# jinhojsk515/spmm

Hardware: AMD Instinct MI355X
Metric: pretrain molecules/sec (higher is better)
Workload: dtype bf16; 1 GPU; SPMM pretrain step, text 12 layers (fusion at 6) + PV 6 layers, H=768, 12 heads, queue 36864, train mode (dropout 0.1), fwd+bwd+clip+AdamW+EMA; global_batch=128, seq_len=128, parallelism=dp1, schedule=eager launches on three HIP streams, packed text rows

## Files before the change

spmm_amd/csrc/gemm.hip:

```cpp
#include "common.h"
#include "../../include/spmm_hip.h"

namespace {

constexpr int BM = 128, BN = 128, BK = 64;
constexpr int TILE_BYTES = BM * BK * 2;
constexpr int STAGE_BYTES = 2 * TILE_BYTES;

enum Epi { EPI_BF16 = 0, EPI_GELU = 1, EPI_F32 = 2, EPI_F32_ATOMIC = 3, EPI_GELU_GRAD = 4, EPI_F32_ACC = 5, EPI_GELU_DERIV = 6, EPI_MUL = 7 };
constexpr bool epi_is_bf16(int e) { return e == EPI_BF16 || e == EPI_GELU || e == EPI_GELU_GRAD || e == EPI_GELU_DERIV || e == EPI_MUL; }

struct GemmP {
  const bf16* A; long lda;
  const bf16* W; long ldw;
  int M, N, K;
  int ksplit;
  const float* bias;
  const float* div_ptr;
  float alpha;
  const bf16* R; long ldr;
  const bf16* G; long ldg;
  void* C; long ldc;
  bf16* C2; long ldc2;
  float* colsum;
// ... 521 lines not shown
        if (p.R) {
          const bf16x4 r = *(const bf16x4*)(p.R + (long)m * p.ldr + n);
#pragma unroll
          for (int j = 0; j < 4; ++j) v[j] += (float)r[j];
        }
        if constexpr (EPI == EPI_BF16) {
          *(bf16x4*)((bf16*)p.C + (long)m * p.ldc + n) = to_bf16x4(v[0], v[1], v[2], v[3]);
        } else if constexpr (EPI == EPI_GELU) {
          *(bf16x4*)(p.C2 + (long)m * p.ldc2 + n) = to_bf16x4(v[0], v[1], v[2], v[3]);
          *(bf16x4*)((bf16*)p.C + (long)m * p.ldc + n) =
              to_bf16x4(gelu_erf(v[0]), gelu_erf(v[1]), gelu_erf(v[2]), gelu_erf(v[3]));
        } else if constexpr (EPI == EPI_GELU_GRAD) {
          const bf16x4 x = *(const bf16x4*)(p.G + (long)m * p.ldg + n);
          *(bf16x4*)((bf16*)p.C + (long)m * p.ldc + n) =
              to_bf16x4(v[0] * gelu_erf_grad((float)x[0]), v[1] * gelu_erf_grad((float)x[1]),
                        v[2] * gelu_erf_grad((float)x[2]), v[3] * gelu_erf_grad((float)x[3]));
        } else if constexpr (EPI == EPI_F32) {
          f32x4 o = {v[0], v[1], v[2], v[3]};
          *(f32x4*)((float*)p.C + (long)m * p.ldc + n) = o;
        } else {
          f32x4* dst = (f32x4*)((float*)p.C + (long)m * p.ldc + n);
          f32x4 o = *dst;
          o[0] += v[0]; o[1] += v[1]; o[2] += v[2]; o[3] += v[3];
          *dst = o;
        }
      }
    }
}

__device__ __forceinline__ void tile_of(int t, int ntm, int ntn, int order, int& tm, int& tn) {
  if (order == 1) { tn = t / ntm; tm = t - tn * ntm; return; }
  if (order == 2) {
    const int gn = (ntn % 4 == 0) ? 4 : (ntn % 3 == 0 ? 3 : (ntn % 2 == 0 ? 2 : 1));
    const int sr = t / (8 * ntn);
    const int rows = min(8, ntm - sr * 8);
    const int r = t - sr * 8 * ntn;
    const int nb = r / (rows * gn), rr = r - nb * rows * gn;
    tm = sr * 8 + rr % rows;
    tn = nb * gn + rr / rows;
    return;
  }
  if (order >= 3 && ntn >= 8) {
    const int ng = order == 3 ? 2 : 4, base = ntn / ng, rem = ntn - base * ng;
    int c0 = 0, u = t;
#pragma unroll
    for (int g = 0; g < 4; ++g) {
      if (g >= ng) break;
      const int cg = base + (g < rem ? 1 : 0), sz = ntm * cg;
      if (u < sz || g == ng - 1) { tm = u / cg; tn = c0 + (u - tm * cg); return; }
      u -= sz; c0 += cg;
    }
  }
  tm = t / ntn; tn = t - tm * ntn;
}

constexpr int BM3 = 256, BN3 = 256;
constexpr int T3_BYTES = 256 * BK * 2;
constexpr int STAGE3_BYTES = 2 * T3_BYTES;
constexpr int LDS3_BYTES = 2 * STAGE3_BYTES;

template <int EPI>
__global__ __launch_bounds__(512) void gemm_nt_v3_kernel(GemmP p) {
  extern __shared__ __attribute__((aligned(16))) char smem3[];
  const int tid = threadIdx.x, lane = tid & 63, wave = tid >> 6;
  const int wm = wave >> 2, wn = wave & 3;
  GEMM_DYN_M(p);
  const int ntm = (p.M + BM3 - 1) / BM3, ntn = (p.N + BN3 - 1) / BN3, nt = ntm * ntn;
  int t;
  {
    const int b = blockIdx.x, q = nt >> 3, r = nt & 7, xcd = b & 7, i = b >> 3;
    if (i >= (xcd < r ? q + 1 : q)) return;
    t = (xcd < r ? xcd * (q + 1) : r * (q + 1) + (xcd - r) * q) + i;
  }
  int tile_m, tile_n;
  tile_of(t, ntm, ntn, p.order, tile_m, tile_n);
  const int m0 = tile_m * BM3, n0 = tile_n * BN3;
  const int nk = p.K / BK;

  f32x16 acc[2][2][2];
#pragma unroll
  for (int h = 0; h < 2; ++h)
#pragma unroll
    for (int i = 0; i < 2; ++i)
#pragma unroll
      for (int j = 0; j < 2; ++j)
#pragma unroll
        for (int r = 0; r < 16; ++r) acc[h][i][j][r] = 0.f;

#define STAGE3(kt_)                                                                           \
  do {                                                                                        \
    char* b_ = smem3 + ((kt_) & 1) * STAGE3_BYTES;                                            \
    stage2_dma(p.A, p.lda, m0, p.M, (kt_) * BK, b_, tid, 4);                                  \
    stage2_dma(p.W, p.ldw, n0, p.N, (kt_) * BK, b_ + T3_BYTES, tid, 4);                       \
  } while (0)

  STAGE3(0);
  for (int kt = 0; kt < nk; ++kt) {
    __syncthreads();
    if (kt + 1 < nk) STAGE3(kt + 1);
    const char* As = smem3 + (kt & 1) * STAGE3_BYTES;
    const char* Ws = As + T3_BYTES;
#pragma unroll
    for (int kk = 0; kk < 4; ++kk) {
      const int s = kk * 2 + (lane >> 5);
      bf16x8 af[4], wf[2];
#pragma unroll
      for (int i = 0; i < 4; ++i) {
        const int ar = wm * 128 + i * 32 + (lane & 31);
        af[i] = *(const bf16x8*)(As + ar * 128 + ((s ^ ((ar >> 1) & 7)) << 4));
      }
#pragma unroll
      for (int i = 0; i < 2; ++i) {
        const int wr = wn * 64 + i * 32 + (lane & 31);
        wf[i] = *(const bf16x8*)(Ws + wr * 128 + ((s ^ ((wr >> 1) & 7)) << 4));
      }
#pragma unroll
      for (int h = 0; h < 2; ++h)
#pragma unroll
        for (int ni = 0; ni < 2; ++ni)
#pragma unroll
          for (int mi = 0; mi < 2; ++mi)
            acc[h][ni][mi] = __builtin_amdgcn_mfma_f32_32x32x16_bf16(wf[ni], af[h * 2 + mi], acc[h][ni][mi], 0, 0, 0);
    }
  }
#undef STAGE3
  __syncthreads();
  char* wt = smem3 + wave * 16384;
  float cs_carry[8] = {0.f, 0.f, 0.f, 0.f, 0.f, 0.f, 0.f, 0.f};
#pragma unroll
  for (int h = 0; h < 2; ++h)
    epilogue_bf16<EPI>(p, acc[h], wt, m0 + wm * 128 + h * 64, n0 + wn * 64, lane, cs_carry, h == 1);
}

constexpr int P8_HT = 128 * BK * 2;
constexpr int P8_BUF = 4 * P8_HT;
constexpr int P8_LDS = 2 * P8_BUF;
constexpr int P8_XLDS = 8 * 4096;

template <int OFF>
__device__ __forceinline__ void p8_dsr(bf16x8& d, uint32_t addr) {
  asm volatile("ds_read_b128 %0, %1 offset:%2" : "=v"(d) : "v"(addr), "n"(OFF) : "memory");
}

struct P8Out { uint32_t d[4]; };
__device__ __forceinline__ uint32_t p8_pack2(float a, float b) {
  typedef __bf16 bf16x2 __attribute__((ext_vector_type(2)));
  bf16x2 v; v[0] = (bf16)a; v[1] = (bf16)b;
  return __builtin_bit_cast(uint32_t, v);
}
__device__ __forceinline__ float p8_lo(uint32_t w) { return __builtin_bit_cast(float, w << 16); }
__device__ __forceinline__ float p8_hi(uint32_t w) { return __builtin_bit_cast(float, w & 0xffff0000u); }
typedef uint32_t u32x2 __attribute__((ext_vector_type(2)));
typedef uint32_t u32x4 __attribute__((ext_vector_type(4)));
template <int OFF>
__device__ __forceinline__ void p8_dsw64(uint32_t addr, uint32_t a, uint32_t b) {
  u32x2 v = {a, b};
  asm volatile("ds_write_b64 %0, %1 offset:%2" :: "v"(addr), "v"(v), "n"(OFF) : "memory");
}
template <int OFF>
__device__ __forceinline__ void p8_dsr128u(u32x4& d, uint32_t addr) {
  asm volatile("ds_read_b128 %0, %1 offset:%2" : "=v"(d) : "v"(addr), "n"(OFF) : "memory");
}

template <int EPI, bool INTERIOR, bool HAS_EX, typename Hook>
__device__ __forceinline__ void p8_epilogue_blocks(const GemmP& p, f32x4 (&acc)[2][4][4], uint32_t xb ,
                                                   int m_base, int n_base, int lane, Hook hook) {
  float scale = p.alpha;
  if (p.div_ptr) scale /= *p.div_ptr;
  const int m = lane & 15, g = lane >> 4, r8 = lane >> 3, c16 = lane & 7;
  f32x4 b[4];
#pragma unroll
  for (int ni = 0; ni < 4; ++ni) b[ni] = f32x4{0.f, 0.f, 0.f, 0.f};
  if (p.bias) {
#pragma unroll
    for (int ni = 0; ni < 4; ++ni)
      if (INTERIOR || n_base + ni * 16 + 4 * g < p.N) b[ni] = *(const f32x4*)(p.bias + n_base + ni * 16 + 4 * g);
  }
  uint32_t wad[4];
#pragma unroll
  for (int ni = 0; ni < 4; ++ni) wad[ni] = xb + (uint32_t)(m * 128 + ((((ni * 2 + (g >> 1)) ^ (m & 7)) << 4) | ((g & 1) << 3)));
  const uint32_t rad = xb + (uint32_t)(r8 * 128 + ((c16 ^ (r8 & 7)) << 4));
  const long n = n_base + c16 * 8;
  const bool n_ok = INTERIOR || n < p.N;
  const long row0 = m_base + r8;
  bf16* cp = (bf16*)p.C + row0 * p.ldc + n;
  constexpr bool GELU2 = EPI == EPI_GELU || EPI == EPI_GELU_DERIV;
  constexpr bool DERIV = EPI == EPI_GELU_DERIV;
  constexpr bool MULG = EPI == EPI_MUL;
  bf16* c2p = GELU2 && p.C2 ? p.C2 + row0 * p.ldc2 + n : nullptr;
  u32x4 ex[8];
  const bf16* esrc = (EPI == EPI_GELU_GRAD || MULG) ? p.G : p.R;
  const long eld = (EPI == EPI_GELU_GRAD || MULG) ? p.ldg : p.ldr;
  const long nn = n_ok ? n : 0;
#define P8_EX_LOAD1(I_, R_)                                                                                            \
  do {                                                                                                                 \
    ex[I_] = *(const u32x4*)(esrc + (R_) * eld + nn);                                                                  \
  } while (0)
#define P8_LOAD_EX(H)                                                          \
  if constexpr (HAS_EX) {                                                      \
    _Pragma("unroll") for (int i_ = 0; i_ < 8; ++i_) {                         \
      long r_ = row0 + (H) * 64 + i_ * 8;                                      \
      if (!INTERIOR) r_ = r_ < p.M ? r_ : p.M - 1;                             \
      P8_EX_LOAD1(i_, r_);                                                     \
    }                                                                          \
  }
  P8_LOAD_EX(0);
  float cs[8] = {0.f, 0.f, 0.f, 0.f, 0.f, 0.f, 0.f, 0.f};
#pragma unroll
  for (int h = 0; h < 2; ++h)
#pragma unroll
    for (int mi = 0; mi < 4; ++mi) {
      const int blk = h * 4 + mi;
      const uint32_t bo = (blk & 1) * 2048;
      const bool ok1 = INTERIOR || (n_ok && row0 + blk * 16 < p.M), ok2 = INTERIOR || (n_ok && row0 + blk * 16 + 8 < p.M);
      float v[4][4];
#pragma unroll
      for (int ni = 0; ni < 4; ++ni)
#pragma unroll
        for (int j = 0; j < 4; ++j) v[ni][j] = acc[h][mi][ni][j] * scale + b[ni][j];
#pragma unroll
      for (int ni = 0; ni < 4; ++ni) acc[h][mi][ni] = f32x4{0.f, 0.f, 0.f, 0.f};
      u32x4 o1, o2;
      if constexpr (GELU2) {
        float w[4][4];
#pragma unroll
        for (int ni = 0; ni < 4; ++ni)
#pragma unroll
          for (int j = 0; j < 4; j += 2) {
            const f32x2 x = {v[ni][j], v[ni][j + 1]};
            f32x2 gg, dd = x;
            gelu_erf_pair<DERIV>(x, gg, dd);
            v[ni][j] = gg.x; v[ni][j + 1] = gg.y;
            w[ni][j] = dd.x; w[ni][j + 1] = dd.y;
          }
        if (c2p) {
          u32x4 q1, q2;
#pragma unroll
          for (int ni = 0; ni < 4; ++ni) p8_dsw64<0>(wad[ni] + bo, p8_pack2(w[ni][0], w[ni][1]), p8_pack2(w[ni][2], w[ni][3]));
#pragma unroll
          for (int ni = 0; ni < 4; ++ni) p8_dsw64<0>(wad[ni] + (bo ^ 2048u), p8_pack2(v[ni][0], v[ni][1]), p8_pack2(v[ni][2], v[ni][3]));
          p8_dsr128u<0>(q1, rad + bo);
          p8_dsr128u<1024>(q2, rad + bo);
          p8_dsr128u<0>(o1, rad + (bo ^ 2048u));
          p8_dsr128u<1024>(o2, rad + (bo ^ 2048u));
          asm volatile("s_waitcnt lgkmcnt(0)" ::: "memory");
          __builtin_amdgcn_sched_barrier(0);
          if (ok1) *(u32x4*)(c2p + (long)blk * 16 * p.ldc2) = q1;
          if (ok2) *(u32x4*)(c2p + (long)blk * 16 * p.ldc2 + 8 * p.ldc2) = q2;
        }
      }
      if (!(GELU2 && c2p)) {
#pragma unroll
        for (int ni = 0; ni < 4; ++ni) p8_dsw64<0>(wad[ni] + bo, p8_pack2(v[ni][0], v[ni][1]), p8_pack2(v[ni][2], v[ni][3]));
        p8_dsr128u<0>(o1, rad + bo);
        p8_dsr128u<1024>(o2, rad + bo);
        asm volatile("s_waitcnt lgkmcnt(0)" ::: "memory");
        __builtin_amdgcn_sched_barrier(0);
      }
      if constexpr (EPI == EPI_BF16 && HAS_EX) {
#pragma unroll
        for (int d = 0; d < 4; ++d) {
          o1[d] = p8_pack2(p8_lo(o1[d]) + p8_lo(ex[2 * mi][d]), p8_hi(o1[d]) + p8_hi(ex[2 * mi][d]));
          o2[d] = p8_pack2(p8_lo(o2[d]) + p8_lo(ex[2 * mi + 1][d]), p8_hi(o2[d]) + p8_hi(ex[2 * mi + 1][d]));
        }
      }
      if constexpr (EPI == EPI_GELU_GRAD) {
#pragma unroll
        for (int d = 0; d < 4; ++d) {
          o1[d] = p8_pack2(p8_lo(o1[d]) * gelu_erf_grad(p8_lo(ex[2 * mi][d])), p8_hi(o1[d]) * gelu_erf_grad(p8_hi(ex[2 * mi][d])));
          o2[d] = p8_pack2(p8_lo(o2[d]) * gelu_erf_grad(p8_lo(ex[2 * mi + 1][d])), p8_hi(o2[d]) * gelu_erf_grad(p8_hi(ex[2 * mi + 1][d])));
        }
      }
      if constexpr (EPI == EPI_MUL) {
#pragma unroll
        for (int d = 0; d < 4; ++d) {
          o1[d] = p8_pack2(p8_lo(o1[d]) * p8_lo(ex[2 * mi][d]), p8_hi(o1[d]) * p8_hi(ex[2 * mi][d]));
          o2[d] = p8_pack2(p8_lo(o2[d]) * p8_lo(ex[2 * mi + 1][d]), p8_hi(o2[d]) * p8_hi(ex[2 * mi + 1][d]));
        }
      }
      if constexpr (!GELU2) {
        if (p.colsum) {
#pragma unroll
          for (int d = 0; d < 4; ++d) {
            if (ok1) { cs[2 * d] += p8_lo(o1[d]); cs[2 * d + 1] += p8_hi(o1[d]); }
            if (ok2) { cs[2 * d] += p8_lo(o2[d]); cs[2 * d + 1] += p8_hi(o2[d]); }
          }
        }
      }
#ifdef P8_NOSTORE
      if (p.M < 0) {
#endif
#ifdef P8_STORE_POLICY
      if (ok1) asm volatile("global_store_dwordx4 %0, %1, off " P8_STORE_POLICY :: "v"(cp + (long)blk * 16 * p.ldc), "v"(o1) : "memory");
      if (ok2) asm volatile("global_store_dwordx4 %0, %1, off " P8_STORE_POLICY :: "v"(cp + (long)blk * 16 * p.ldc + 8 * p.ldc), "v"(o2) : "memory");
#else
      if (ok1) *(u32x4*)(cp + (long)blk * 16 * p.ldc) = o1;
      if (ok2) *(u32x4*)(cp + (long)blk * 16 * p.ldc + 8 * p.ldc) = o2;
#endif
#ifdef P8_NOSTORE
      }
#endif
      hook(blk);
      if constexpr (HAS_EX && EPI == EPI_GELU_GRAD) {
        if (blk == 3) { P8_LOAD_EX(1); }
      } else if constexpr (HAS_EX) {
        if (h == 0) {
#pragma unroll
          for (int i_ = 2 * mi; i_ < 2 * mi + 2; ++i_) {
            long r_ = row0 + 64 + i_ * 8;
            if (!INTERIOR) r_ = r_ < p.M ? r_ : p.M - 1;
            P8_EX_LOAD1(i_, r_);
          }
        }
      }
    }
#undef P8_LOAD_EX
#undef P8_EX_LOAD1
  if constexpr (!GELU2) {
    if (p.colsum) {
#pragma unroll
      for (int e = 0; e < 8; ++e) {
        float t = cs[e];
        t += __shfl_xor(t, 8, 64);
        t += __shfl_xor(t, 16, 64);
        t += __shfl_xor(t, 32, 64);
        cs[e] = t;
      }
      if (lane < 8 && n_ok) {
#pragma unroll
        for (int e = 0; e < 8; ++e) atomicAdd(p.colsum + n + e, cs[e]);
      }
    }
  }
}

template <int EPI>
__global__ __launch_bounds__(512) void gemm_nt_p8_kernel(GemmP p) {
  extern __shared__ __attribute__((aligned(16))) char smem8[];
  const int tid = threadIdx.x, lane = tid & 63;
  const int wave = __builtin_amdgcn_readfirstlane(tid >> 6);
  const int wr = wave >> 2, wc = wave & 3;
  GEMM_DYN_M(p);
  const int ntm = (p.M + BM3 - 1) / BM3, ntn = (p.N + BN3 - 1) / BN3, nt = ntm * ntn;
  if ((int)blockIdx.x >= nt) return;
  const int nk = p.K / BK;

  f32x4 acc[2][4][4];
#define P8_ZERO()                                                              \
  _Pragma("unroll") for (int h_ = 0; h_ < 2; ++h_)                             \
  _Pragma("unroll") for (int i_ = 0; i_ < 4; ++i_)                             \
  _Pragma("unroll") for (int j_ = 0; j_ < 4; ++j_) acc[h_][i_][j_] = f32x4{0.f, 0.f, 0.f, 0.f}
  P8_ZERO();

  uint32_t offA[2][2], offW[2][2];
  const uint32_t ls16 = (uint32_t)(((tid & 7) ^ ((tid >> 4) & 7)) * 16);
  int m0, n0;
#define P8_TILE(VB)                                                                                           \
  do {                                                                                                        \
    const int b_ = (VB), q_ = nt >> 3, r_ = nt & 7, xcd_ = b_ & 7, i_ = b_ >> 3;                              \
    const int t_ = (xcd_ < r_ ? xcd_ * (q_ + 1) : r_ * (q_ + 1) + (xcd_ - r_) * q_) + i_;                     \
    int tm_, tn_;                                                                                             \
    tile_of(t_, ntm, ntn, p.order, tm_, tn_);                                                                 \
    m0 = tm_ * BM3; n0 = tn_ * BN3;                                                                           \
    _Pragma("unroll") for (int h_ = 0; h_ < 2; ++h_)                                                          \
    _Pragma("unroll") for (int j_ = 0; j_ < 2; ++j_) {                                                        \
      int row_ = m0 + j_ * 128 + h_ * 64 + (tid >> 3);                                                        \
      row_ = row_ < p.M ? row_ : p.M - 1;                     \
      offA[h_][j_] = (uint32_t)row_ * (uint32_t)(p.lda * 2) + ls16;                                                      \
      int col_ = n0 + (j_ * 2 + (tid >> 8)) * 64 + h_ * 32 + ((tid >> 3) & 31);                               \
      col_ = col_ < p.N ? col_ : p.N - 1;                                                                     \
      offW[h_][j_] = (uint32_t)col_ * (uint32_t)(p.ldw * 2) + ls16;                                                      \
    }                                                                                                         \
  } while (0)
  const char* gA = (const char*)p.A;
  const char* gW = (const char*)p.W;
  const uint32_t lds0 = (uint32_t)(uintptr_t)(LDS_AS char*)smem8;
#define P8_STG(GB, O, SLOT)                                                                                               \
  do {                                                                                                                    \
    const uint32_t d_ = lds0 + (SLOT) + wave * 1024;                                                                      \
    asm volatile("s_mov_b32 m0, %2\n\ts_nop 0\n\tglobal_load_lds_dwordx4 %0, %1" :: "v"((O)[0]), "s"(GB), "s"(d_) : "memory", "m0");          \
    asm volatile("s_mov_b32 m0, %2\n\ts_nop 0\n\tglobal_load_lds_dwordx4 %0, %1" :: "v"((O)[1]), "s"(GB), "s"(d_ + 8192) : "memory", "m0");   \
  } while (0)
#define P8_STG_A(H, BUF, KT) P8_STG((const char*)(gA + (size_t)(KT) * (BK * 2)), offA[H], (BUF) * P8_BUF + (H) * P8_HT)
#define P8_STG_W(H, BUF, KT) P8_STG((const char*)(gW + (size_t)(KT) * (BK * 2)), offW[H], (BUF) * P8_BUF + (2 + (H)) * P8_HT)
#define P8_PROLOGUE()                                                                        \
  do {                                                                                       \
    P8_STG_A(0, 0, 0); P8_STG_W(0, 0, 0); P8_STG_W(1, 0, 0); P8_STG_A(1, 0, 0);              \
    P8_STG_W(0, 1, 1); P8_STG_A(0, 1, 1); P8_STG_W(1, 1, 1);                                 \
  } while (0)

  uint32_t aad[2][2], wad[2][2];
  {
    const uint32_t sw = (uint32_t)((lane >> 1) & 7), r16 = (uint32_t)(lane & 15), q = (uint32_t)(lane >> 4);
#pragma unroll
    for (int kk = 0; kk < 2; ++kk) {
      const uint32_t slot = ((((uint32_t)kk * 4 + q) ^ sw) << 4);
      aad[0][kk] = lds0 + ((uint32_t)wr * 64 + r16) * 128 + slot;
      wad[0][kk] = lds0 + 2 * P8_HT + ((uint32_t)wc * 32 + r16) * 128 + slot;
      aad[1][kk] = aad[0][kk] + P8_BUF;
      wad[1][kk] = wad[0][kk] + P8_BUF;
    }
  }
  bf16x8 fa[4][2], fw0[2][2], fw1[2][2];
#define P8_RD_A(BUF, H)                                                                       \
  do {                                                                                        \
    p8_dsr<(H) * P8_HT + 0 * 2048>(fa[0][0], aad[BUF][0]);                                    \
    p8_dsr<(H) * P8_HT + 1 * 2048>(fa[1][0], aad[BUF][0]);                                    \
    p8_dsr<(H) * P8_HT + 2 * 2048>(fa[2][0], aad[BUF][0]);                                    \
    p8_dsr<(H) * P8_HT + 3 * 2048>(fa[3][0], aad[BUF][0]);                                    \
    p8_dsr<(H) * P8_HT + 0 * 2048>(fa[0][1], aad[BUF][1]);                                    \
    p8_dsr<(H) * P8_HT + 1 * 2048>(fa[1][1], aad[BUF][1]);                                    \
    p8_dsr<(H) * P8_HT + 2 * 2048>(fa[2][1], aad[BUF][1]);                                    \
    p8_dsr<(H) * P8_HT + 3 * 2048>(fa[3][1], aad[BUF][1]);                                    \
  } while (0)
#define P8_RD_W(BUF, H, FW)                                                                   \
  do {                                                                                        \
    p8_dsr<(H) * P8_HT + 0 * 2048>(FW[0][0], wad[BUF][0]);                                    \
    p8_dsr<(H) * P8_HT + 1 * 2048>(FW[1][0], wad[BUF][0]);                                    \
    p8_dsr<(H) * P8_HT + 0 * 2048>(FW[0][1], wad[BUF][1]);                                    \
    p8_dsr<(H) * P8_HT + 1 * 2048>(FW[1][1], wad[BUF][1]);                                    \
  } while (0)
#define P8_MM(H, NH, FW)                                                                                        \
  do {                                                                                                          \
    _Pragma("unroll") for (int kk_ = 0; kk_ < 2; ++kk_)                                                         \
    _Pragma("unroll") for (int mi_ = 0; mi_ < 4; ++mi_)                                                         \
    _Pragma("unroll") for (int ni_ = 0; ni_ < 2; ++ni_)                                                         \
      acc[H][mi_][(NH) * 2 + ni_] =                                                                             \
          __builtin_amdgcn_mfma_f32_16x16x32_bf16(FW[ni_][kk_], fa[mi_][kk_], acc[H][mi_][(NH) * 2 + ni_], 0, 0, 0); \
  } while (0)
#define P8_BAR() __builtin_amdgcn_s_barrier()
#define P8_SB() __builtin_amdgcn_sched_barrier(0)
#define P8_LGKM0() asm volatile("s_waitcnt lgkmcnt(0)" ::: "memory")
#define P8_COMPUTE(H, NH, FW)                    \
  do {                                           \
    P8_BAR();                                    \
    P8_LGKM0();                                  \
    P8_SB();                                     \
    __builtin_amdgcn_s_setprio(1);               \
    P8_MM(H, NH, FW);                            \
    __builtin_amdgcn_s_setprio(0);               \
    P8_SB();                                     \
    P8_BAR();                                    \
    P8_SB();                                     \
  } while (0)

#ifdef P8_PROFILE
  unsigned long long* prof = (unsigned long long*)p.colsum + (size_t)blockIdx.x * 16 * 8;
  p.colsum = nullptr;
  int prof_i = 0;
#define P8_STAMP(K) do { if (prof && tid == 0 && prof_i < 16) prof[prof_i * 8 + (K)] = __builtin_readcyclecounter(); } while (0)
#else
#define P8_STAMP(K) do { } while (0)
#endif
  int vb = blockIdx.x;
  bool pre = false;
  P8_TILE(vb);
  P8_PROLOGUE();
  asm volatile("s_waitcnt vmcnt(6)" ::: "memory");
  P8_BAR();
  P8_SB();
  if (wr == 1) P8_BAR();
  for (;;) {
    P8_STAMP(0);
    const int cm0 = m0, cn0 = n0;
    const int vbn = vb + (int)gridDim.x;
    const bool has_next = vbn < nt;
    const bool pre_next = has_next && cm0 + BM3 <= p.M && cn0 + BN3 <= p.N;
    for (int kt = 0; kt < nk; kt += 2) {
      const bool last = kt + 2 >= nk;
      const bool more = !last || has_next;
      int kn = kt + 2;
      P8_RD_W(0, 0, fw0); P8_SB(); P8_RD_A(0, 0);
      if (!(pre && kt == 0)) P8_STG_A(1, 1, kt + 1);
      asm volatile("s_waitcnt lgkmcnt(8)" ::: "memory");
      P8_COMPUTE(0, 0, fw0);
      if (last && has_next) { P8_TILE(vbn); kn = 0; }
      P8_RD_W(0, 1, fw1);
      if (more) P8_STG_W(0, 0, kn);
      P8_COMPUTE(0, 1, fw1);
      P8_RD_A(0, 1);
      if (more) P8_STG_A(0, 0, kn);
      P8_COMPUTE(1, 1, fw1);
      if (more) {
        P8_STG_W(1, 0, kn);
        if (pre && kt == 0) asm volatile("s_waitcnt vmcnt(22)" ::: "memory");
        else asm volatile("s_waitcnt vmcnt(6)" ::: "memory");
      } else {
        asm volatile("s_waitcnt vmcnt(0)" ::: "memory");
      }
      P8_COMPUTE(1, 0, fw0);
      P8_RD_W(1, 0, fw0); P8_SB(); P8_RD_A(1, 0);
      if (more) P8_STG_A(1, 0, kn);
      asm volatile("s_waitcnt lgkmcnt(8)" ::: "memory");
      P8_COMPUTE(0, 0, fw0);
      P8_RD_W(1, 1, fw1);
      if (more) P8_STG_W(0, 1, kn + 1);
      P8_COMPUTE(0, 1, fw1);
      P8_RD_A(1, 1);
      if (more) P8_STG_A(0, 1, kn + 1);
      P8_COMPUTE(1, 1, fw1);
      if (more) {
        P8_STG_W(1, 1, kn + 1);
        if (last && pre_next) {
          P8_STG_A(1, 1, kn + 1);
          asm volatile("s_waitcnt vmcnt(8)" ::: "memory");
        } else {
          asm volatile("s_waitcnt vmcnt(6)" ::: "memory");
        }
      }
      P8_COMPUTE(1, 0, fw0);
    }
    P8_STAMP(2);

    if (wr == 0) P8_BAR();
    P8_SB();
    {
      int lane_e = lane;
      asm volatile("" : "+v"(lane_e));
      GemmP q = p;
      asm volatile("" : "+s"(q.C), "+s"(q.ldc), "+s"(q.C2), "+s"(q.ldc2));
      asm volatile("" : "+s"(q.R), "+s"(q.ldr), "+s"(q.G), "+s"(q.ldg));
      asm volatile("" : "+s"(q.bias), "+s"(q.colsum), "+s"(q.div_ptr), "+s"(q.alpha), "+s"(q.M), "+s"(q.N));
      auto hook = [](int) {};
      const uint32_t xb = lds0 + P8_LDS + wave * 4096;
      const int mb = cm0 + wr * 128, nb = cn0 + wc * 64;
      const bool interior = cm0 + BM3 <= q.M && cn0 + BN3 <= q.N;
      if constexpr (EPI == EPI_GELU_GRAD || EPI == EPI_MUL) {
        if (interior) p8_epilogue_blocks<EPI, true, true>(q, acc, xb, mb, nb, lane_e, hook);
        else p8_epilogue_blocks<EPI, false, true>(q, acc, xb, mb, nb, lane_e, hook);
      } else if (EPI == EPI_BF16 && q.R != nullptr) {
        if (interior) p8_epilogue_blocks<EPI, true, true>(q, acc, xb, mb, nb, lane_e, hook);
        else p8_epilogue_blocks<EPI, false, true>(q, acc, xb, mb, nb, lane_e, hook);
      } else {
        if (interior) p8_epilogue_blocks<EPI, true, false>(q, acc, xb, mb, nb, lane_e, hook);
        else p8_epilogue_blocks<EPI, false, false>(q, acc, xb, mb, nb, lane_e, hook);
      }
    }
    P8_SB();
    if (wr == 1) P8_BAR();
    P8_STAMP(4);
#ifdef P8_PROFILE
    ++prof_i;
#endif
    if (!has_next) break;
    vb = vbn;
    pre = pre_next;
    P8_SB();
  }
  if (wr == 0) P8_BAR();
#undef P8_ZERO
#undef P8_STAMP
#undef P8_TILE
#undef P8_PROLOGUE
#undef P8_STG
#undef P8_STG_A
#undef P8_STG_W
#undef P8_RD_A
#undef P8_RD_W
#undef P8_MM
#undef P8_COMPUTE
#undef P8_BAR
#undef P8_SB
#undef P8_LGKM0
}

template <typename K>
int raise_lds(K kernel, int bytes, const char* what) {
  hipError_t e = hipFuncSetAttribute((const void*)kernel, hipFuncAttributeMaxDynamicSharedMemorySize, bytes);
  if (e != hipSuccess) {
    spmm_set_error("spmm_gemm_nt: cannot raise the dynamic LDS of %s to %d: %s", what, bytes, hipGetErrorString(e));
    return SPMM_ERR_LAUNCH;
  }
  return SPMM_OK;
}

template <int EPI>
int launch_p8_one(const GemmP& p, hipStream_t st, bool persist) {
  static const int rc = raise_lds(gemm_nt_p8_kernel<EPI>, P8_LDS + P8_XLDS, "the 8-phase kernel");
  if (rc != SPMM_OK) return rc;
  const int nt = ((p.M + BM3 - 1) / BM3) * ((p.N + BN3 - 1) / BN3);
  static const int ncu = [] { int dev = 0, n = 0; (void)hipGetDevice(&dev); (void)hipDeviceGetAttribute(&n, hipDeviceAttributeMultiprocessorCount, dev); return n > 0 ? n & ~7 : 256; }();
  dim3 grid(persist && nt > ncu ? ncu : nt);
  hipLaunchKernelGGL((gemm_nt_p8_kernel<EPI>), grid, dim3(512), P8_LDS + P8_XLDS, st, p);
  return SPMM_OK;
}
int launch_p8(int epi, const GemmP& p, hipStream_t st, bool persist) {
  switch (epi) {
    case EPI_BF16: return launch_p8_one<EPI_BF16>(p, st, persist);
    case EPI_GELU: return launch_p8_one<EPI_GELU>(p, st, persist);
    case EPI_GELU_GRAD: return launch_p8_one<EPI_GELU_GRAD>(p, st, persist);
    case EPI_GELU_DERIV: return launch_p8_one<EPI_GELU_DERIV>(p, st, persist);
    case EPI_MUL: return launch_p8_one<EPI_MUL>(p, st, persist);
    default: return -1;
  }
}

template <int EPI>
int launch_v3_one(const GemmP& p, hipStream_t st) {
  static const int rc = raise_lds(gemm_nt_v3_kernel<EPI>, LDS3_BYTES, "the 256x256 kernel");
  if (rc != SPMM_OK) return rc;
  dim3 grid(((p.M + BM3 - 1) / BM3) * ((p.N + BN3 - 1) / BN3));
  hipLaunchKernelGGL((gemm_nt_v3_kernel<EPI>), grid, dim3(512), LDS3_BYTES, st, p);
  return SPMM_OK;
}
int launch_v3(int epi, const GemmP& p, hipStream_t st) {
  switch (epi) {
    case EPI_BF16: return launch_v3_one<EPI_BF16>(p, st);
    case EPI_GELU: return launch_v3_one<EPI_GELU>(p, st);
    case EPI_GELU_GRAD: return launch_v3_one<EPI_GELU_GRAD>(p, st);
    case EPI_GELU_DERIV: return launch_v3_one<EPI_GELU_DERIV>(p, st);
    case EPI_MUL: return launch_v3_one<EPI_MUL>(p, st);
    default: return -1;
  }
}

template <int EPI>
int launch_v2_one(const GemmP& p, hipStream_t st) {
  static const int rc = raise_lds(gemm_nt_v2_kernel<EPI>, LDS2_BYTES, "the 256x128 kernel");
  if (rc != SPMM_OK) return rc;
  dim3 grid(((p.M + BM2 - 1) / BM2) * ((p.N + BN - 1) / BN));
  hipLaunchKernelGGL((gemm_nt_v2_kernel<EPI>), grid, dim3(512), LDS2_BYTES, st, p);
  return SPMM_OK;
}
int launch_v2(int epi, const GemmP& p, hipStream_t st) {
  switch (epi) {
    case EPI_BF16: return launch_v2_one<EPI_BF16>(p, st);
    case EPI_GELU: return launch_v2_one<EPI_GELU>(p, st);
    case EPI_F32: return launch_v2_one<EPI_F32>(p, st);
    case EPI_GELU_GRAD: return launch_v2_one<EPI_GELU_GRAD>(p, st);
    case EPI_GELU_DERIV: return launch_v2_one<EPI_GELU_DERIV>(p, st);
    case EPI_MUL: return launch_v2_one<EPI_MUL>(p, st);
    case EPI_F32_ACC: return launch_v2_one<EPI_F32_ACC>(p, st);
    default: return -1;
  }
}

template <typename K>
int pc_attr(K kernel) {
  static const hipError_t e = hipFuncSetAttribute((const void*)kernel, hipFuncAttributeMaxDynamicSharedMemorySize, PC_LDS);
  return e == hipSuccess ? 0 : 1;
}
#define PC_LAUNCH(E)                                                                                   \
  case E:                                                                                              \
    if (pc_attr(gemm_nt_pc_kernel<E>)) { spmm_set_error("spmm_gemm_nt: cannot raise the LDS limit of the loader/compute kernel"); return SPMM_ERR_LAUNCH; } \
    hipLaunchKernelGGL((gemm_nt_pc_kernel<E>), grid, dim3(PC_THREADS), PC_LDS, st, p);                        \
    break
int launch_pc(int epi, const GemmP& p, dim3 grid, hipStream_t st) {
  switch (epi) {
    PC_LAUNCH(EPI_BF16); PC_LAUNCH(EPI_GELU); PC_LAUNCH(EPI_F32); PC_LAUNCH(EPI_F32_ATOMIC); PC_LAUNCH(EPI_GELU_GRAD); PC_LAUNCH(EPI_F32_ACC);
    PC_LAUNCH(EPI_GELU_DERIV); PC_LAUNCH(EPI_MUL);
    default: return -1;
  }
  return 0;
}
#undef PC_LAUNCH

int launch_v1(int epi, const GemmP& p, dim3 grid, hipStream_t st) {
  switch (epi) {
    case EPI_BF16: hipLaunchKernelGGL((gemm_nt_kernel<EPI_BF16>), grid, dim3(256), 0, st, p); break;
    case EPI_GELU: hipLaunchKernelGGL((gemm_nt_kernel<EPI_GELU>), grid, dim3(256), 0, st, p); break;
    case EPI_F32: hipLaunchKernelGGL((gemm_nt_kernel<EPI_F32>), grid, dim3(256), 0, st, p); break;
    case EPI_F32_ATOMIC: hipLaunchKernelGGL((gemm_nt_kernel<EPI_F32_ATOMIC>), grid, dim3(256), 0, st, p); break;
    case EPI_GELU_GRAD: hipLaunchKernelGGL((gemm_nt_kernel<EPI_GELU_GRAD>), grid, dim3(256), 0, st, p); break;
    case EPI_F32_ACC: hipLaunchKernelGGL((gemm_nt_kernel<EPI_F32_ACC>), grid, dim3(256), 0, st, p); break;
    case EPI_GELU_DERIV: hipLaunchKernelGGL((gemm_nt_kernel<EPI_GELU_DERIV>), grid, dim3(256), 0, st, p); break;
    case EPI_MUL: hipLaunchKernelGGL((gemm_nt_kernel<EPI_MUL>), grid, dim3(256), 0, st, p); break;
    default: return -1;
  }
  return SPMM_OK;
}

inline bool is_bf16_epi(int epi) { return epi_is_bf16(epi); }
inline bool p8_ok(const GemmP& p, int epi) {
  return is_bf16_epi(epi) && p.K % 128 == 0 && p.N % 8 == 0 && (unsigned long)p.M * (unsigned long)p.lda * 2ul < (1ul << 32) &&
         (unsigned long)p.N * (unsigned long)p.ldw * 2ul < (1ul << 32);
}

int pick_tile(int M, int N, int epi) {
  const bool bf = is_bf16_epi(epi);
  if (M >= 6000) {
    const long t3 = (long)((M + 255) / 256) * ((N + 255) / 256);
    if (bf && t3 >= 96) return 3;
    return (epi != EPI_F32_ATOMIC) ? 2 : 1;
  }
  auto tiles = [&](int bm, int bn) { return (double)((M + bm - 1) / bm) * ((N + bn - 1) / bn); };
  auto fill = [](double t) { const double w = (double)(long)((t + 255) / 256); return t / (256.0 * w); };
  const double t3 = tiles(256, 256), t2 = tiles(256, 128), t1 = tiles(128, 128);
  const double s3 = bf ? 1.20 * fill(t3) : 0.0;
  const double s2 = (M >= 512 && epi != EPI_F32_ATOMIC) ? 0.85 * fill(t2) : 0.0;
  const double s1 = 0.80 * (t1 < 256 ? t1 / 256.0 : 1.0);
  if (s3 >= s2 && s3 >= s1) return 3;
  return s2 >= s1 ? 2 : 1;
}

}

extern "C" int spmm_gemm_nt(const void* A, long lda, const void* W, long ldw, int M, int N, int K, int splits,
                            const float* bias, const float* div_ptr, float alpha, const void* R, long ldr,
                            const void* G, long ldg, void* C, long ldc, void* C2, long ldc2, int epi, float* colsum,
                            int kernel, const int* M_dev, hipStream_t stream) {
  SPMM_CHECK_SHAPE(M > 0 && N > 0 && K > 0, "spmm_gemm_nt: empty problem M=%d N=%d K=%d", M, N, K);
  SPMM_CHECK_SHAPE(K % 64 == 0, "spmm_gemm_nt: K=%d must be a multiple of 64", K);
  SPMM_CHECK_SHAPE(N % 4 == 0, "spmm_gemm_nt: N=%d must be a multiple of 4", N);
  SPMM_CHECK_SHAPE(lda % 8 == 0 && ldw % 8 == 0, "spmm_gemm_nt: lda/ldw must be multiples of 8 elements");
  SPMM_CHECK_SHAPE(ldc % 4 == 0, "spmm_gemm_nt: ldc must be a multiple of 4");
  SPMM_CHECK_SHAPE(!is_bf16_epi(epi) || (ldc % 8 == 0 && (!R || ldr % 8 == 0) && (!G || ldg % 8 == 0) && (!C2 || ldc2 % 8 == 0) && (uintptr_t)C % 16 == 0),
                   "spmm_gemm_nt: bf16 outputs need 16-B aligned rows (ldc/ldr/ldg/ldc2 multiples of 8)");
  SPMM_CHECK_SHAPE(((uintptr_t)A % 16 == 0) && ((uintptr_t)W % 16 == 0), "spmm_gemm_nt: A/W must be 16-B aligned");
  SPMM_CHECK_SHAPE(epi >= EPI_BF16 && epi <= EPI_MUL, "spmm_gemm_nt: unknown epilogue %d", epi);
  if (splits < 1) splits = 1;
  SPMM_CHECK_SHAPE(splits == 1 || epi == EPI_F32_ATOMIC, "spmm_gemm_nt: split-K needs the atomic epilogue");
  SPMM_CHECK_SHAPE((epi != EPI_GELU_GRAD && epi != EPI_MUL) || G != nullptr, "spmm_gemm_nt: the GELU-grad / multiply epilogues need G");
  SPMM_CHECK_SHAPE(colsum == nullptr || epi == EPI_BF16 || epi == EPI_GELU_GRAD || epi == EPI_MUL, "spmm_gemm_nt: colsum is only fused into the bf16 / GELU-grad / multiply epilogues");
  int ksplit = ((K / 64 + splits - 1) / splits) * 64;
  splits = (K + ksplit - 1) / ksplit;
  GemmP p;
  p.A = (const bf16*)A; p.lda = lda; p.W = (const bf16*)W; p.ldw = ldw;
  p.M = M; p.N = N; p.K = K; p.ksplit = ksplit; p.bias = bias; p.div_ptr = div_ptr; p.alpha = alpha;
  p.R = (const bf16*)R; p.ldr = ldr; p.G = (const bf16*)G; p.ldg = ldg; p.C = C; p.ldc = ldc;
  p.C2 = (bf16*)C2; p.ldc2 = ldc2; p.colsum = colsum;
  p.M_ptr = nullptr;
  p.order = K > 1024 ? 0 : 2;

  int k = kernel == SPMM_GEMM_AUTO_TILES ? 0 : kernel;
  if (k == 0) {
    const int tile = splits > 1 ? 1 : pick_tile(M, N, epi);
    k = tile == 3 ? (p8_ok(p, epi) ? (kernel == SPMM_GEMM_AUTO_TILES ? 9 : 8) : 3) : tile;
    if (k == 2 && (epi == EPI_F32_ATOMIC || M < 512)) k = 1;
  }
  const bool pc_fits = (unsigned long)p.M * (unsigned long)p.lda * 2ul < (1ul << 32) && (unsigned long)p.N * (unsigned long)p.ldw * 2ul < (1ul << 32);
  const long t128 = (long)((M + BM - 1) / BM) * ((N + BN - 1) / BN) * splits;
  if (k == 1 && kernel != 1 && pc_fits && PC_AUTO && t128 <= 256 && ksplit >= 4 * BK) k = 5;
  SPMM_CHECK_SHAPE(k == 1 || k == 2 || k == 3 || k == 5 || k == 8 || k == 9, "spmm_gemm_nt: unknown kernel selector %d", kernel);
  SPMM_CHECK_SHAPE(k != 5 || pc_fits, "spmm_gemm_nt: kernel 5 addresses its operands with 32-bit byte offsets (< 4 GiB each)");
  SPMM_CHECK_SHAPE((k != 8 && k != 9) || p8_ok(p, epi), "spmm_gemm_nt: the 8-phase kernel needs a bf16-output epilogue, K %% 128 == 0, N %% 8 == 0 and operands < 4 GiB");
  SPMM_CHECK_SHAPE(k != 3 || is_bf16_epi(epi), "spmm_gemm_nt: the 256x256 kernel has bf16-output epilogues only");
  SPMM_CHECK_SHAPE(k != 2 || epi != EPI_F32_ATOMIC, "spmm_gemm_nt: the 256x128 kernel has no atomic epilogue");
  SPMM_CHECK_SHAPE(k == 1 || k == 5 || splits == 1, "spmm_gemm_nt: split-K runs on the 128x128 kernels only");
  p.M_ptr = M_dev;
  int rc;
  if (k == 8 || k == 9) rc = launch_p8(epi, p, stream, k == 8);
  else if (k == 3) rc = launch_v3(epi, p, stream);
  else if (k == 2) rc = launch_v2(epi, p, stream);
  else if (k == 5) rc = launch_pc(epi, p, dim3(((M + BM - 1) / BM) * ((N + BN - 1) / BN), 1, splits), stream);
  else rc = launch_v1(epi, p, dim3(((M + BM - 1) / BM) * ((N + BN - 1) / BN), 1, splits), stream);
  if (rc > 0) return rc;
  if (rc < 0) { spmm_set_error("spmm_gemm_nt: epilogue %d is not built for kernel %d", epi, k); return SPMM_ERR_UNSUPPORTED; }
  SPMM_LAUNCH_CHECK("spmm_gemm_nt");
  return SPMM_OK;
}
```

Measured before the change: 2388 molecules/s.

## Software-pipeline the 8-phase GEMM epilogue LDS round trips across row blocks

Restructures the 8-phase GEMM epilogue so the arithmetic and LDS write/read transpose for the next 16-row block are issued before waiting on the current block, using double-buffered registers and partial lgkmcnt waits. Only the GELU-grad path keeps the old serial form. Global loads and stores now go through explicit global address-space pointers so the compiler can emit global instead of flat instructions. It also adds an optional workgroup cap for the persistent kernel, encoded in the high bits of the kernel selector, plus profiling hooks. The extra live registers for the double buffers could lower occupancy or cause spills.

```diff
diff --git a/spmm_amd/csrc/gemm.hip b/spmm_amd/csrc/gemm.hip
--- a/spmm_amd/csrc/gemm.hip
+++ b/spmm_amd/csrc/gemm.hip
@@ -697,6 +697,12 @@
 __device__ __forceinline__ float p8_hi(uint32_t w) { return __builtin_bit_cast(float, w & 0xffff0000u); }
 typedef uint32_t u32x2 __attribute__((ext_vector_type(2)));
 typedef uint32_t u32x4 __attribute__((ext_vector_type(4)));
+#ifdef P8_FLAT_IO
+#define P8_GLOBAL
+#else
+#define P8_GLOBAL __attribute__((address_space(1)))
+#endif
+__device__ __forceinline__ void p8_gstore(bf16* ptr, u32x4 v) { *(P8_GLOBAL u32x4*)ptr = v; }
 template <int OFF>
 __device__ __forceinline__ void p8_dsw64(uint32_t addr, uint32_t a, uint32_t b) {
   u32x2 v = {a, b};
@@ -739,7 +745,7 @@
   const long nn = n_ok ? n : 0;
 #define P8_EX_LOAD1(I_, R_)                                                                                            \
   do {                                                                                                                 \
-    ex[I_] = *(const u32x4*)(esrc + (R_) * eld + nn);                                                                  \
+    ex[I_] = *(const P8_GLOBAL u32x4*)(esrc + (R_) * eld + nn);                           \
   } while (0)
 #define P8_LOAD_EX(H)                                                          \
   if constexpr (HAS_EX) {                                                      \
@@ -751,114 +757,196 @@
   }
   P8_LOAD_EX(0);
   float cs[8] = {0.f, 0.f, 0.f, 0.f, 0.f, 0.f, 0.f, 0.f};
-#pragma unroll
-  for (int h = 0; h < 2; ++h)
-#pragma unroll
-    for (int mi = 0; mi < 4; ++mi) {
-      const int blk = h * 4 + mi;
+  uint32_t pk[2][8], pk2[2][8];
+  u32x4 o1[2], o2[2], q1, q2;
+  auto arith = [&](int blk, bool two) __attribute__((always_inline)) {
+    const int h = blk >> 2, mi = blk & 3, s = blk & 1;
+    float v[4][4];
+#pragma unroll
+    for (int ni = 0; ni < 4; ++ni)
+#pragma unroll
+      for (int j = 0; j < 4; ++j) v[ni][j] = acc[h][mi][ni][j] * scale + b[ni][j];
+#pragma unroll
+    for (int ni = 0; ni < 4; ++ni) acc[h][mi][ni] = f32x4{0.f, 0.f, 0.f, 0.f};
+    if constexpr (GELU2) {
+      float w[4][4];
+#pragma unroll
+      for (int ni = 0; ni < 4; ++ni)
+#pragma unroll
+        for (int j = 0; j < 4; j += 2) {
+          const f32x2 x = {v[ni][j], v[ni][j + 1]};
+          f32x2 gg, dd = x;
+          gelu_erf_pair<DERIV>(x, gg, dd);
+          v[ni][j] = gg.x; v[ni][j + 1] = gg.y;
+          w[ni][j] = dd.x; w[ni][j + 1] = dd.y;
+        }
+      if (two) {
+#pragma unroll
+        for (int ni = 0; ni < 4; ++ni) { pk2[s][ni * 2] = p8_pack2(w[ni][0], w[ni][1]); pk2[s][ni * 2 + 1] = p8_pack2(w[ni][2], w[ni][3]); }
+      }
+    }
+#pragma unroll
+    for (int ni = 0; ni < 4; ++ni) { pk[s][ni * 2] = p8_pack2(v[ni][0], v[ni][1]); pk[s][ni * 2 + 1] = p8_pack2(v[ni][2], v[ni][3]); }
+  };
+  auto trip1 = [&](int blk) __attribute__((always_inline)) {
+    const int s = blk & 1;
+    const uint32_t bo = s * 2048;
+#pragma unroll
+    for (int ni = 0; ni < 4; ++ni) p8_dsw64<0>(wad[ni] + bo, pk[s][ni * 2], pk[s][ni * 2 + 1]);
+    p8_dsr128u<0>(o1[s], rad + bo);
+    p8_dsr128u<1024>(o2[s], rad + bo);
+  };
+  auto trip2 = [&](int blk) __attribute__((always_inline)) {
+    const int s = blk & 1;
+    const uint32_t bo = s * 2048;
+#pragma unroll
+    for (int ni = 0; ni < 4; ++ni) p8_dsw64<0>(wad[ni] + bo, pk2[s][ni * 2], pk2[s][ni * 2 + 1]);
+#pragma unroll
+    for (int ni = 0; ni < 4; ++ni) p8_dsw64<0>(wad[ni] + (bo ^ 2048u), pk[s][ni * 2], pk[s][ni * 2 + 1]);
+    p8_dsr128u<0>(q1, rad + bo);
+    p8_dsr128u<1024>(q2, rad + bo);
+    p8_dsr128u<0>(o1[s], rad + (bo ^ 2048u));
+    p8_dsr128u<1024>(o2[s], rad + (bo ^ 2048u));
+  };
+  auto finish = [&](int blk, bool ok1, bool ok2) __attribute__((always_inline)) {
+    const int h = blk >> 2, mi = blk & 3, s = blk & 1;
+    (void)h;
+    u32x4 a1 = o1[s], a2 = o2[s];
+    if constexpr (EPI == EPI_BF16 && HAS_EX) {
+#pragma unroll
+      for (int d = 0; d < 4; ++d) {
+        a1[d] = p8_pack2(p8_lo(a1[d]) + p8_lo(ex[2 * mi][d]), p8_hi(a1[d]) + p8_hi(ex[2 * mi][d]));
+        a2[d] = p8_pack2(p8_lo(a2[d]) + p8_lo(ex[2 * mi + 1][d]), p8_hi(a2[d]) + p8_hi(ex[2 * mi + 1][d]));
+      }
+    }
+    if constexpr (EPI == EPI_MUL) {
+#pragma unroll
+      for (int d = 0; d < 4; ++d) {
+        a1[d] = p8_pack2(p8_lo(a1[d]) * p8_lo(ex[2 * mi][d]), p8_hi(a1[d]) * p8_hi(ex[2 * mi][d]));
+        a2[d] = p8_pack2(p8_lo(a2[d]) * p8_lo(ex[2 * mi + 1][d]), p8_hi(a2[d]) * p8_hi(ex[2 * mi + 1][d]));
+      }
+    }
+    if constexpr (!GELU2) {
+      if (p.colsum) {
+#pragma unroll
+        for (int d = 0; d < 4; ++d) {
+          if (ok1) { cs[2 * d] += p8_lo(a1[d]); cs[2 * d + 1] += p8_hi(a1[d]); }
+          if (ok2) { cs[2 * d] += p8_lo(a2[d]); cs[2 * d + 1] += p8_hi(a2[d]); }
+        }
+      }
+    }
+#ifdef P8_NOSTORE
+    if (p.M < 0) {
+#endif
+#ifdef P8_STORE_POLICY
+    if (ok1) asm volatile("global_store_dwordx4 %0, %1, off " P8_STORE_POLICY :: "v"(cp + (long)blk * 16 * p.ldc), "v"(a1) : "memory");
+    if (ok2) asm volatile("global_store_dwordx4 %0, %1, off " P8_STORE_POLICY :: "v"(cp + (long)blk * 16 * p.ldc + 8 * p.ldc), "v"(a2) : "memory");
+#else
+    if (ok1) p8_gstore(cp + (long)blk * 16 * p.ldc, a1);
+    if (ok2) p8_gstore(cp + (long)blk * 16 * p.ldc + 8 * p.ldc, a2);
+#endif
+#ifdef P8_NOSTORE
+    }
+#endif
+    hook(blk);
+    if constexpr (HAS_EX) {
+      if (h == 0) {
+#pragma unroll
+        for (int i_ = 2 * mi; i_ < 2 * mi + 2; ++i_) {
+          long r_ = row0 + 64 + i_ * 8;
+          if (!INTERIOR) r_ = r_ < p.M ? r_ : p.M - 1;
+          P8_EX_LOAD1(i_, r_);
+        }
+      }
+    }
+  };
+#define P8_LWAIT(N, X, Y) asm volatile("s_waitcnt lgkmcnt(" #N ")" : "+v"(X), "+v"(Y) :: "memory")
+  if (GELU2 && c2p) {
+    arith(0, true);
+#pragma unroll
+    for (int blk = 0; blk < 8; ++blk) {
+      const int s = blk & 1;
+      trip2(blk);
+      __builtin_amdgcn_sched_barrier(0);
+      if (blk < 7) arith(blk + 1, true);
+      __builtin_amdgcn_sched_barrier(0);
+      P8_LWAIT(2, q1, q2);
+      __builtin_amdgcn_sched_barrier(0);
+      const bool ok1 = INTERIOR || (n_ok && row0 + blk * 16 < p.M), ok2 = INTERIOR || (n_ok && row0 + blk * 16 + 8 < p.M);
+      if (ok1) p8_gstore(c2p + (long)blk * 16 * p.ldc2, q1);
+      if (ok2) p8_gstore(c2p + (long)blk * 16 * p.ldc2 + 8 * p.ldc2, q2);
+      P8_LWAIT(0, o1[s], o2[s]);
+      __builtin_amdgcn_sched_barrier(0);
+      finish(blk, ok1, ok2);
+    }
+  } else if constexpr (EPI == EPI_GELU_GRAD) {
+#pragma unroll
+    for (int blk = 0; blk < 8; ++blk) {
+      const int mi = blk & 3;
       const uint32_t bo = (blk & 1) * 2048;
       const bool ok1 = INTERIOR || (n_ok && row0 + blk * 16 < p.M), ok2 = INTERIOR || (n_ok && row0 + blk * 16 + 8 < p.M);
       float v[4][4];
 #pragma unroll
       for (int ni = 0; ni < 4; ++ni)
 #pragma unroll
-        for (int j = 0; j < 4; ++j) v[ni][j] = acc[h][mi][ni][j] * scale + b[ni][j];
-#pragma unroll
-      for (int ni = 0; ni < 4; ++ni) acc[h][mi][ni] = f32x4{0.f, 0.f, 0.f, 0.f};
-      u32x4 o1, o2;
-      if constexpr (GELU2) {
-        float w[4][4];
-#pragma unroll
-        for (int ni = 0; ni < 4; ++ni)
-#pragma unroll
-          for (int j = 0; j < 4; j += 2) {
-            const f32x2 x = {v[ni][j], v[ni][j + 1]};
-            f32x2 gg, dd = x;
-            gelu_erf_pair<DERIV>(x, gg, dd);
-            v[ni][j] = gg.x; v[ni][j + 1] = gg.y;
-            w[ni][j] = dd.x; w[ni][j + 1] = dd.y;
-          }
-        if (c2p) {
-          u32x4 q1, q2;
-#pragma unroll
-          for (int ni = 0; ni < 4; ++ni) p8_dsw64<0>(wad[ni] + bo, p8_pack2(w[ni][0], w[ni][1]), p8_pack2(w[ni][2], w[ni][3]));
-#pragma unroll
-          for (int ni = 0; ni < 4; ++ni) p8_dsw64<0>(wad[ni] + (bo ^ 2048u), p8_pack2(v[ni][0], v[ni][1]), p8_pack2(v[ni][2], v[ni][3]));
-          p8_dsr128u<0>(q1, rad + bo);
-          p8_dsr128u<1024>(q2, rad + bo);
-          p8_dsr128u<0>(o1, rad + (bo ^ 2048u));
-          p8_dsr128u<1024>(o2, rad + (bo ^ 2048u));
-          asm volatile("s_waitcnt lgkmcnt(0)" ::: "memory");
-          __builtin_amdgcn_sched_barrier(0);
-          if (ok1) *(u32x4*)(c2p + (long)blk * 16 * p.ldc2) = q1;
-          if (ok2) *(u32x4*)(c2p + (long)blk * 16 * p.ldc2 + 8 * p.ldc2) = q2;
-        }
-      }
-      if (!(GELU2 && c2p)) {
-#pragma unroll
-        for (int ni = 0; ni < 4; ++ni) p8_dsw64<0>(wad[ni] + bo, p8_pack2(v[ni][0], v[ni][1]), p8_pack2(v[ni][2], v[ni][3]));
-        p8_dsr128u<0>(o1, rad + bo);
-        p8_dsr128u<1024>(o2, rad + bo);
-        asm volatile("s_waitcnt lgkmcnt(0)" ::: "memory");
-        __builtin_amdgcn_sched_barrier(0);
-      }
-      if constexpr (EPI == EPI_BF16 && HAS_EX) {
+        for (int j = 0; j < 4; ++j) v[ni][j] = acc[blk >> 2][mi][ni][j] * scale + b[ni][j];
+#pragma unroll
+      for (int ni = 0; ni < 4; ++ni) acc[blk >> 2][mi][ni] = f32x4{0.f, 0.f, 0.f, 0.f};
+      u32x4 g1, g2;
+#pragma unroll
+      for (int ni = 0; ni < 4; ++ni) p8_dsw64<0>(wad[ni] + bo, p8_pack2(v[ni][0], v[ni][1]), p8_pack2(v[ni][2], v[ni][3]));
+      p8_dsr128u<0>(g1, rad + bo);
+      p8_dsr128u<1024>(g2, rad + bo);
+      asm volatile("s_waitcnt lgkmcnt(0)" ::: "memory");
+      __builtin_amdgcn_sched_barrier(0);
+#pragma unroll
+      for (int d = 0; d < 4; ++d) {
+        g1[d] = p8_pack2(p8_lo(g1[d]) * gelu_erf_grad(p8_lo(ex[2 * mi][d])), p8_hi(g1[d]) * gelu_erf_grad(p8_hi(ex[2 * mi][d])));
+        g2[d] = p8_pack2(p8_lo(g2[d]) * gelu_erf_grad(p8_lo(ex[2 * mi + 1][d])), p8_hi(g2[d]) * gelu_erf_grad(p8_hi(ex[2 * mi + 1][d])));
+      }
+      if (p.colsum) {
 #pragma unroll
         for (int d = 0; d < 4; ++d) {
-          o1[d] = p8_pack2(p8_lo(o1[d]) + p8_lo(ex[2 * mi][d]), p8_hi(o1[d]) + p8_hi(ex[2 * mi][d]));
-          o2[d] = p8_pack2(p8_lo(o2[d]) + p8_lo(ex[2 * mi + 1][d]), p8_hi(o2[d]) + p8_hi(ex[2 * mi + 1][d]));
-        }
-      }
-      if constexpr (EPI == EPI_GELU_GRAD) {
-#pragma unroll
-        for (int d = 0; d < 4; ++d) {
-          o1[d] = p8_pack2(p8_lo(o1[d]) * gelu_erf_grad(p8_lo(ex[2 * mi][d])), p8_hi(o1[d]) * gelu_erf_grad(p8_hi(ex[2 * mi][d])));
-          o2[d] = p8_pack2(p8_lo(o2[d]) * gelu_erf_grad(p8_lo(ex[2 * mi + 1][d])), p8_hi(o2[d]) * gelu_erf_grad(p8_hi(ex[2 * mi + 1][d])));
-        }
-      }
-      if constexpr (EPI == EPI_MUL) {
-#pragma unroll
-        for (int d = 0; d < 4; ++d) {
-          o1[d] = p8_pack2(p8_lo(o1[d]) * p8_lo(ex[2 * mi][d]), p8_hi(o1[d]) * p8_hi(ex[2 * mi][d]));
-          o2[d] = p8_pack2(p8_lo(o2[d]) * p8_lo(ex[2 * mi + 1][d]), p8_hi(o2[d]) * p8_hi(ex[2 * mi + 1][d]));
-        }
-      }
-      if constexpr (!GELU2) {
-        if (p.colsum) {
-#pragma unroll
-          for (int d = 0; d < 4; ++d) {
-            if (ok1) { cs[2 * d] += p8_lo(o1[d]); cs[2 * d + 1] += p8_hi(o1[d]); }
-            if (ok2) { cs[2 * d] += p8_lo(o2[d]); cs[2 * d + 1] += p8_hi(o2[d]); }
-          }
+          if (ok1) { cs[2 * d] += p8_lo(g1[d]); cs[2 * d + 1] += p8_hi(g1[d]); }
+          if (ok2) { cs[2 * d] += p8_lo(g2[d]); cs[2 * d + 1] += p8_hi(g2[d]); }
         }
       }
 #ifdef P8_NOSTORE
       if (p.M < 0) {
 #endif
 #ifdef P8_STORE_POLICY
-      if (ok1) asm volatile("global_store_dwordx4 %0, %1, off " P8_STORE_POLICY :: "v"(cp + (long)blk * 16 * p.ldc), "v"(o1) : "memory");
-      if (ok2) asm volatile("global_store_dwordx4 %0, %1, off " P8_STORE_POLICY :: "v"(cp + (long)blk * 16 * p.ldc + 8 * p.ldc), "v"(o2) : "memory");
+      if (ok1) asm volatile("global_store_dwordx4 %0, %1, off " P8_STORE_POLICY :: "v"(cp + (long)blk * 16 * p.ldc), "v"(g1) : "memory");
+      if (ok2) asm volatile("global_store_dwordx4 %0, %1, off " P8_STORE_POLICY :: "v"(cp + (long)blk * 16 * p.ldc + 8 * p.ldc), "v"(g2) : "memory");
 #else
-      if (ok1) *(u32x4*)(cp + (long)blk * 16 * p.ldc) = o1;
-      if (ok2) *(u32x4*)(cp + (long)blk * 16 * p.ldc + 8 * p.ldc) = o2;
+      if (ok1) p8_gstore(cp + (long)blk * 16 * p.ldc, g1);
+      if (ok2) p8_gstore(cp + (long)blk * 16 * p.ldc + 8 * p.ldc, g2);
 #endif
 #ifdef P8_NOSTORE
       }
 #endif
       hook(blk);
-      if constexpr (HAS_EX && EPI == EPI_GELU_GRAD) {
-        if (blk == 3) { P8_LOAD_EX(1); }
-      } else if constexpr (HAS_EX) {
-        if (h == 0) {
-#pragma unroll
-          for (int i_ = 2 * mi; i_ < 2 * mi + 2; ++i_) {
-            long r_ = row0 + 64 + i_ * 8;
-            if (!INTERIOR) r_ = r_ < p.M ? r_ : p.M - 1;
-            P8_EX_LOAD1(i_, r_);
-          }
-        }
-      }
-    }
+      if (blk == 3) { P8_LOAD_EX(1); }
+    }
+  } else {
+    arith(0, false);
+    trip1(0);
+#pragma unroll
+    for (int blk = 0; blk < 8; ++blk) {
+      const int s = blk & 1;
+      __builtin_amdgcn_sched_barrier(0);
+      if (blk < 7) {
+        arith(blk + 1, false);
+        trip1(blk + 1);
+        P8_LWAIT(6, o1[s], o2[s]);
+      } else {
+        P8_LWAIT(0, o1[s], o2[s]);
+      }
+      __builtin_amdgcn_sched_barrier(0);
+      const bool ok1 = INTERIOR || (n_ok && row0 + blk * 16 < p.M), ok2 = INTERIOR || (n_ok && row0 + blk * 16 + 8 < p.M);
+      finish(blk, ok1, ok2);
+    }
+  }
+#undef P8_LWAIT
 #undef P8_LOAD_EX
 #undef P8_EX_LOAD1
   if constexpr (!GELU2) {
@@ -1066,7 +1154,12 @@
       asm volatile("" : "+s"(q.C), "+s"(q.ldc), "+s"(q.C2), "+s"(q.ldc2));
       asm volatile("" : "+s"(q.R), "+s"(q.ldr), "+s"(q.G), "+s"(q.ldg));
       asm volatile("" : "+s"(q.bias), "+s"(q.colsum), "+s"(q.div_ptr), "+s"(q.alpha), "+s"(q.M), "+s"(q.N));
+#ifdef P8_PROFILE
+      P8_STAMP(1);
+      auto hook = [&](int blk) { if (blk == 0) P8_STAMP(5); if (blk == 6) P8_STAMP(3); };
+#else
       auto hook = [](int) {};
+#endif
       const uint32_t xb = lds0 + P8_LDS + wave * 4096;
       const int mb = cm0 + wr * 128, nb = cn0 + wc * 64;
       const bool interior = cm0 + BM3 <= q.M && cn0 + BN3 <= q.N;
@@ -1120,22 +1213,22 @@
 }
 
 template <int EPI>
-int launch_p8_one(const GemmP& p, hipStream_t st, bool persist) {
+int launch_p8_one(const GemmP& p, hipStream_t st, bool persist, int cap) {
   static const int rc = raise_lds(gemm_nt_p8_kernel<EPI>, P8_LDS + P8_XLDS, "the 8-phase kernel");
   if (rc != SPMM_OK) return rc;
   const int nt = ((p.M + BM3 - 1) / BM3) * ((p.N + BN3 - 1) / BN3);
   static const int ncu = [] { int dev = 0, n = 0; (void)hipGetDevice(&dev); (void)hipDeviceGetAttribute(&n, hipDeviceAttributeMultiprocessorCount, dev); return n > 0 ? n & ~7 : 256; }();
-  dim3 grid(persist && nt > ncu ? ncu : nt);
+  dim3 grid(persist && cap > 0 ? (nt < cap ? nt : cap) : (persist && nt > ncu ? ncu : nt));
   hipLaunchKernelGGL((gemm_nt_p8_kernel<EPI>), grid, dim3(512), P8_LDS + P8_XLDS, st, p);
   return SPMM_OK;
 }
-int launch_p8(int epi, const GemmP& p, hipStream_t st, bool persist) {
+int launch_p8(int epi, const GemmP& p, hipStream_t st, bool persist, int cap) {
   switch (epi) {
-    case EPI_BF16: return launch_p8_one<EPI_BF16>(p, st, persist);
-    case EPI_GELU: return launch_p8_one<EPI_GELU>(p, st, persist);
-    case EPI_GELU_GRAD: return launch_p8_one<EPI_GELU_GRAD>(p, st, persist);
-    case EPI_GELU_DERIV: return launch_p8_one<EPI_GELU_DERIV>(p, st, persist);
-    case EPI_MUL: return launch_p8_one<EPI_MUL>(p, st, persist);
+    case EPI_BF16: return launch_p8_one<EPI_BF16>(p, st, persist, cap);
+    case EPI_GELU: return launch_p8_one<EPI_GELU>(p, st, persist, cap);
+    case EPI_GELU_GRAD: return launch_p8_one<EPI_GELU_GRAD>(p, st, persist, cap);
+    case EPI_GELU_DERIV: return launch_p8_one<EPI_GELU_DERIV>(p, st, persist, cap);
+    case EPI_MUL: return launch_p8_one<EPI_MUL>(p, st, persist, cap);
     default: return -1;
   }
 }
@@ -1267,6 +1360,9 @@
   p.M_ptr = nullptr;
   p.order = K > 1024 ? 0 : 2;
 
+  const int p8_cap = kernel >= 256 ? kernel >> 8 : 0;
+  if (p8_cap) kernel &= 255;
+  SPMM_CHECK_SHAPE(p8_cap == 0 || kernel == SPMM_GEMM_K256P8, "spmm_gemm_nt: a workgroup cap goes with the persistent 8-phase kernel only");
   int k = kernel == SPMM_GEMM_AUTO_TILES ? 0 : kernel;
   if (k == 0) {
     const int tile = splits > 1 ? 1 : pick_tile(M, N, epi);
@@ -1284,7 +1380,7 @@
   SPMM_CHECK_SHAPE(k == 1 || k == 5 || splits == 1, "spmm_gemm_nt: split-K runs on the 128x128 kernels only");
   p.M_ptr = M_dev;
   int rc;
-  if (k == 8 || k == 9) rc = launch_p8(epi, p, stream, k == 8);
+  if (k == 8 || k == 9) rc = launch_p8(epi, p, stream, k == 8, p8_cap);
   else if (k == 3) rc = launch_v3(epi, p, stream);
   else if (k == 2) rc = launch_v2(epi, p, stream);
   else if (k == 5) rc = launch_pc(epi, p, dim3(((M + BM - 1) / BM) * ((N + BN - 1) / BN), 1, splits), stream);
```

After: 2412 molecules/s (median of 6 runs). No clear change (+1.0%).
